# luanaruiz9/gated_gcrnns

Measured on AMD Instinct MI355X. Metric: sequences/sec (node), N=1000 K=5 T=32 F=64, higher is better.
Workload: dtype bf16

## Files before the change

### gated_gcrnns_amd/csrc/gcrnn_fused_seq32.h

```cpp
#pragma once

#if defined(GCRNN_SEQ_STAMPS)
static __device__ unsigned long long gcrnn_seq32_stamps[256 * 96];
static __device__ __forceinline__ void gcrnn_stamp32_put(uint32_t lds_addr) {
  const unsigned long long tv = __builtin_amdgcn_s_memtime();
  asm volatile("ds_write_b64 %0, %1" ::"v"(lds_addr), "v"(tv) : "memory");
}
static __device__ __forceinline__ unsigned long long gcrnn_stamp32_get(uint32_t lds_addr) {
  unsigned long long tv;
  asm volatile("ds_read_b64 %0, %1\n\ts_waitcnt lgkmcnt(0)" : "=v"(tv) : "v"(lds_addr) : "memory");
  return tv;
}
#define GCRNN_STAMP32(slot)                                                                                   \
  do {                                                                                                        \
    if (wave == 0 && stamp_on && lane_now() == 0) gcrnn_stamp32_put((uint32_t)reinterpret_cast<uintptr_t>(smem) + M::FLAG_OFF + 8 * (slot)); \
  } while (0)
#define GCRNN_STAMP32_WAVE(slot0)                                                                             \
  do {                                                                                                        \
    if (stamp_on && lane_now() == 0) gcrnn_stamp32_put((uint32_t)reinterpret_cast<uintptr_t>(smem) + M::FLAG_OFF + 8 * ((slot0) + wave)); \
  } while (0)
#define GCRNN_STAMP32_FLUSH()                                                                                 \
  do {                                                                                                        \
    __syncthreads();                                                                                          \
    if (threadIdx.x < 96 && blockIdx.x < 256) gcrnn_seq32_stamps[blockIdx.x * 96 + threadIdx.x] = gcrnn_stamp32_get((uint32_t)reinterpret_cast<uintptr_t>(smem) + M::FLAG_OFF + 8 * threadIdx.x); \
// ... 197 lines not shown
          const bool ok = nodes[i] < N;
          const int nn = ok ? nodes[i] : 0;
          const char* ra = smem + (8 * qo) * SROW + ((((nn >> 3) + 2 * qo) & 127) << 4) + (nn & 7) * 2;
          uint32_t h16[8];
#pragma unroll
          for (int j = 0; j < 8; ++j) h16[j] = *reinterpret_cast<const uint16_t*>(ra + j * SROW);
          typedef __attribute__((__vector_size__(4 * sizeof(unsigned int)))) unsigned int u32x4s_t;
          u32x4s_t v;
#pragma unroll
          for (int jj = 0; jj < 4; ++jj) v[jj] = ok ? (h16[2 * jj] | (h16[2 * jj + 1] << 16)) : 0u;
          bfr[i][s] = __builtin_bit_cast(bf16x8, v);
        }
        lds_barrier();
      }
      if (a.nsteps > 1) {
        constexpr int XN = RPH * NPCK, XROWS = G, XPPR = XN / 8, XPCS = XROWS / 8;
        static_assert(XROWS * XN * 2 <= 32 * SROW && (XROWS * XPPR) % STHREADS == 0 && (XPCS * XN) % STHREADS == 0 && XPPR >= 16, "x_1 start-up rounds");
        const __amdgpu_buffer_rsrc_t rsrc_x1 = __builtin_amdgcn_make_buffer_rsrc(a.pk_dst0 + a.pkdst_stride + (int64_t)b * (NP * G), 0, NP * G * 2, 0x00020000);
        const uint16_t* src = a.pk_src0 + (int64_t)b * a.pk_stride + a.pksrc_stride;
#pragma unroll
        for (int i = 0; i < XROWS * XPPR / STHREADS; ++i) {
          const int id = i * STHREADS + tl;
          const int row = id / XPPR, cs = id - row * XPPR;
          const int col = (cs - 2 * (row >> 3) + XPPR) % XPPR;
          if (col * 8 < N)
            __builtin_amdgcn_global_load_lds((const __attribute__((address_space(1))) void*)(src + (int64_t)row * N + col * 8),
                                             (__attribute__((address_space(3))) void*)(smem + (i * STHREADS + wave * 64) * 16), 16, 0, GCRNN_SEQ32_NT_DMA);
        }
        asm volatile("s_waitcnt vmcnt(0)" ::: "memory");
        lds_barrier();
        constexpr int XRI = XPCS * XN / STHREADS;
        typedef __attribute__((__vector_size__(4 * sizeof(unsigned int)))) unsigned int u32x4x_t;
        u32x4x_t vv[XRI];
#pragma unroll
        for (int i = 0; i < XRI; ++i) {
          const int id = i * STHREADS + tl;
          const int nl = id / XPCS, pc = id - nl * XPCS;
          const char* ra = smem + (8 * pc) * (XN * 2) + ((((nl >> 3) + 2 * pc) % XPPR) << 4) + (nl & 7) * 2;
          uint32_t h16[8];
#pragma unroll
          for (int j = 0; j < 8; ++j) h16[j] = *reinterpret_cast<const uint16_t*>(ra + j * (XN * 2));
          const bool ok = nl < N;
#pragma unroll
          for (int jj = 0; jj < 4; ++jj) vv[i][jj] = ok ? (h16[2 * jj] | (h16[2 * jj + 1] << 16)) : 0u;
        }
#pragma unroll
        for (int i = 0; i < XRI; ++i) asm volatile("" : "+v"(vv[i]));
#pragma unroll
        for (int i = 0; i < XRI; ++i) {
          const int id = i * STHREADS + tl;
          const int nl = id / XPCS, pc = id - nl * XPCS;
          __builtin_amdgcn_raw_buffer_store_b128(vv[i], rsrc_x1, nl * (G * 2) + pc * 16, 0, 0);
        }
        asm volatile("s_waitcnt vmcnt(0)" ::: "memory");
#pragma unroll
        for (int i = 0; i < XRI; ++i) asm volatile("" ::"v"(vv[i]));
        lds_barrier();
      }
    }
  }

  int tbeg[STILES], tend[STILES];
#pragma unroll
  for (int i = 0; i < STILES; ++i) {
    tbeg[i] = a.tile_off[wave * STILES + i];
    tend[i] = a.tile_off[wave * STILES + i + 1];
  }
  char* wtab = smem + COL_OFF + entries * 32 + GCRNN_HOP_COLUMN_PAD;
  for (int idx = tid; idx < NP; idx += STHREADS) reinterpret_cast<int32_t*>(wtab)[idx] = a.tile_nodes[idx];
  [[maybe_unused]] float* r1tab = reinterpret_cast<float*>(wtab + NP * 4);
  if constexpr (R1) {
    for (int idx = tid; idx < NP; idx += STHREADS) {
      const int nd = a.tile_nodes[idx] >> 16;
      r1tab[idx] = nd < NP ? a.r1a[nd] : 0.f;
      r1tab[NP + idx] = nd < NP ? a.r1b[nd] : 0.f;
    }
  }
  auto slot_words = [&](int ln, int (&w)[STILES]) {
    const uint32_t ad = (uint32_t)(COL_OFF + entries * 32 + GCRNN_HOP_COLUMN_PAD) + (uint32_t)((wave * STILES * 16 + (ln & 15)) * 4);
    asm volatile("ds_read_b32 %0, %8\n\tds_read_b32 %1, %8 offset:64\n\tds_read_b32 %2, %8 offset:128\n\tds_read_b32 %3, %8 offset:192\n\t"
                 "ds_read_b32 %4, %8 offset:256\n\tds_read_b32 %5, %8 offset:320\n\tds_read_b32 %6, %8 offset:384\n\tds_read_b32 %7, %8 offset:448\n\t"
                 "s_waitcnt lgkmcnt(0)"
                 : "=&v"(w[0]), "=&v"(w[1]), "=&v"(w[2]), "=&v"(w[3]), "=&v"(w[4]), "=&v"(w[5]), "=&v"(w[6]), "=&v"(w[7])
                 : "v"(ad));
    const int lb = (((ln >> 4) >> 1) << 4) | (((ln >> 4) & 1) << 3);
#pragma unroll
    for (int i = 0; i < STILES; ++i) w[i] ^= lb;
  };
  [[maybe_unused]] auto r1_scale = [&](f32x4 (&ac)[STILES][2], int kind) __attribute__((always_inline)) {
    if constexpr (R1) {
      const uint32_t ad = (uint32_t)(COL_OFF + entries * 32 + GCRNN_HOP_COLUMN_PAD + NP * 4 + NP * 4) + (uint32_t)((wave * STILES * 16 + (lane_now() & 15)) * 4);
      constexpr int NB = (GATED || ITEMS || K == 4) ? 1 : 4;
#pragma unroll
      for (int h4 = 0; h4 < STILES; h4 += NB) {
        float b4[NB];
        if constexpr (NB == 4)
          asm volatile("ds_read_b32 %0, %4\n\tds_read_b32 %1, %4 offset:64\n\tds_read_b32 %2, %4 offset:128\n\tds_read_b32 %3, %4 offset:192\n\t"
                       "s_waitcnt lgkmcnt(0)"
                       : "=&v"(b4[0]), "=&v"(b4[1]), "=&v"(b4[2]), "=&v"(b4[3])
                       : "v"(ad + (uint32_t)(h4 * 64)));
        else
          asm volatile("ds_read_b32 %0, %1\n\ts_waitcnt lgkmcnt(0)" : "=&v"(b4[0]) : "v"(ad + (uint32_t)(h4 * 64)));
#pragma unroll
        for (int e = 0; e < NB; ++e) {
          const float bv = b4[e];
          const float f = kind == 0 ? bv : (bv == 0.f ? 1.f : (kind == 1 ? __builtin_amdgcn_rcpf(bv) : bv));
          ac[h4 + e][0] *= f; ac[h4 + e][1] *= f;
        }
      }
    }
  };

  {
    const int cbytes = entries * 32;
    const char* csrc = reinterpret_cast<const char*>(a.ell_col4);
    for (int p = wave; p * 1024 < cbytes; p += SWAVES)
      if (p * 1024 + lane * 16 < cbytes)
        __builtin_amdgcn_global_load_lds((const __attribute__((address_space(1))) void*)(csrc + p * 1024 + lane * 16),
                                         (__attribute__((address_space(3))) void*)(smem + COL_OFF + p * 1024), 16, 0, 0);
    const char* wsrc = reinterpret_cast<const char*>(a.wpack) + (size_t)chunk0 * WB;
    for (int p = wave; p < WB / 1024; p += SWAVES)
      __builtin_amdgcn_global_load_lds((const __attribute__((address_space(1))) void*)(wsrc + p * 1024 + lane * 16),
                                       (__attribute__((address_space(3))) void*)(smem + WOFF + p * 1024), 16, 0, 0);
    asm volatile("s_waitcnt vmcnt(0)" ::: "memory");
  }
  if (tid < GCRNN_HOP_COLUMN_PAD / 4) reinterpret_cast<uint32_t*>(smem + COL_OFF + entries * 32)[tid] = 0u;
  float* lbias = reinterpret_cast<float*>(smem + M::BIAS_OFF);
  if constexpr (UPR1) {
    if (tid < F) lbias[tid] = a.head_w[tid];
  } else
  if (tid < NCH * 32) lbias[tid] = a.bias ? a.bias[tid] : 0.f;
  if constexpr (HEADV) {
    float* ht = reinterpret_cast<float*>(smem + COL_OFF + entries * 32 + GCRNN_HOP_COLUMN_PAD + NP * 4 + (R1 ? 2 * NP * 4 : 0));
    if (tid < F) ht[tid] = a.head_w[tid];
    if (tid == F) ht[64] = a.head_b ? a.head_b[0] : 0.f;
  }
  __syncthreads();

  if (a.stagger > 0) {
    const unsigned long long t0 = __builtin_amdgcn_s_memtime();
    const unsigned long long d = (unsigned long long)((blockIdx.x >> 3) & 7) * (unsigned long long)a.stagger;
    while (__builtin_amdgcn_s_memtime() - t0 < d) __builtin_amdgcn_s_sleep(16);
  }
  const uint32_t lds0 = (uint32_t)reinterpret_cast<uintptr_t>(smem);
  if (lds0 != 0) __builtin_trap();
  const uint32_t lds_col = lds0 + COL_OFF;
  [[maybe_unused]] float* htab = reinterpret_cast<float*>(wtab + NP * 4 + (R1 ? 2 * NP * 4 : 0));
  char* xtile = wtab + NP * 4 + (R1 ? 2 * NP * 4 : 0) + (HEADV ? M::HEAD_TAB : 0);

  const int skip_hi = __builtin_amdgcn_readfirstlane((MODE == 3 || (MODE == 1 && a.flags && a.flags[0] != 0)) ? 1 : 0);
  const bool skip_h = skip_hi != 0;
  auto load_first_operand = [&](int b) {
    const __amdgpu_buffer_rsrc_t rsrc_h = __builtin_amdgcn_make_buffer_rsrc(const_cast<uint16_t*>(a.hfirst), 0, skip_h ? 0 : (ITEMS ? a.hmod : B) * (NP * F * 2), 0x00020000);
    const __amdgpu_buffer_rsrc_t rsrc_x = __builtin_amdgcn_make_buffer_rsrc(const_cast<uint16_t*>(a.x0), 0, XS > 0 ? B * (NP * G * 2) : 0, 0x00020000);
    const int bh = ITEMS ? __builtin_amdgcn_readfirstlane(b % a.hmod) : b;
    const int ln0 = lane_now(), qo = ln0 >> 4;
    int sw[STILES];
    slot_words(ln0, sw);
#pragma unroll
    for (int s = 0; s < KS; ++s) {
#pragma unroll
      for (int i = 0; i < STILES; ++i) {
        const int w = sw[i];
        if (s < HS)
          bfr[i][s] = __builtin_bit_cast(bf16x8, __builtin_amdgcn_raw_buffer_load_b128(rsrc_h, (w >> 16) * (F * 2) + 16 * qo + 64 * s, bh * (NP * F * 2), 0));
        else
          bfr[i][s] = __builtin_bit_cast(bf16x8, __builtin_amdgcn_raw_buffer_load_b128(rsrc_x, (w >> 16) * (G * 2) + 16 * qo + 64 * (s - HS), b * (NP * G * 2), 0));
      }
    }
  };
  bool have_operand = self_start;
  for (int b = wg_seq; b < B; b += gseq) {
  if (!have_operand) load_first_operand(b);
  have_operand = false;
#pragma unroll 1
  for (int step = 0; step < a.nsteps; ++step) {
    const bool fin = (MODE == 2) && a.final_raw && step == a.nsteps - 1;
    uint16_t* hout = fin ? a.final_out : (a.out0 ? a.out0 + (int64_t)step * a.ostride : nullptr);
    [[maybe_unused]] const uint16_t* ep_dh = (SONLY && !fin && a.dh0_) ? a.dh0_ + (int64_t)step * a.dhstride : nullptr;
    [[maybe_unused]] const float* ep_ng = (MODE == 4) ? a.ng0 + (int64_t)step * a.ngstride : nullptr;
    [[maybe_unused]] const uint16_t* ep_h = (MODE == 2) ? (fin ? a.final_h : (a.hs0 ? a.hs0 + (int64_t)step * a.hsstride : nullptr)) : nullptr;
    [[maybe_unused]] const uint16_t* ep_dy = (UPR1 && !fin && a.dy0) ? a.dy0 + (int64_t)step * a.dystride + (int64_t)b * a.dybstride : nullptr;
    [[maybe_unused]] const bool ep_up = UPR1 ? ep_dy != nullptr : ep_dh != nullptr;
    [[maybe_unused]] float* gpart = (MODE == 2 && a.gpart0) ? a.gpart0 + (int64_t)step * a.gpartstride : nullptr;
    [[maybe_unused]] float gsc = 1.f;
    if constexpr (MODE == 2) {
      if (a.gsc0) gsc = __builtin_bit_cast(float, __builtin_amdgcn_readfirstlane(__builtin_bit_cast(int, a.gsc0[(int64_t)step * a.gscstride + b])));
    }
    float gin = 1.f, gfo = 1.f, gratio = 1.f;
    if constexpr (MODE == 4) {
      if (a.gi0) {
        gin = __builtin_bit_cast(float, __builtin_amdgcn_readfirstlane(__builtin_bit_cast(int, a.gi0[(int64_t)step * a.gstride + b])));
        gfo = __builtin_bit_cast(float, __builtin_amdgcn_readfirstlane(__builtin_bit_cast(int, a.gf0[(int64_t)step * a.gstride + b])));
      }
    }
    if constexpr (GATED) {
      gin = __builtin_bit_cast(float, __builtin_amdgcn_readfirstlane(__builtin_bit_cast(int, a.gi0[(int64_t)step * a.gstride + b])));
      gfo = __builtin_bit_cast(float, __builtin_amdgcn_readfirstlane(__builtin_bit_cast(int, a.gf0[(int64_t)step * a.gstride + b])));
      gratio = __builtin_bit_cast(float, __builtin_amdgcn_readfirstlane(__builtin_bit_cast(int, gfo / fmaxf(gin, 1e-30f))));
    }
    const uint16_t* aux1 = (USERV && a.a1) ? (a.a1_last_only ? (step == a.nsteps - 1 ? a.a1 : nullptr) : a.a1 + (int64_t)step * a.a1stride) : nullptr;
    const bool pk_any = PKV && a.pk_src0 != nullptr;
    const int ubstride = a.ubstride;
    const int nb = b + (int)gridDim.x;
    const int nbq = ITEMS ? __builtin_amdgcn_readfirstlane(nb / a.hmod) : 0, nbr = ITEMS ? __builtin_amdgcn_readfirstlane(nb - nbq * a.hmod) : 0;
    const int64_t pk_soff = ITEMS ? (int64_t)nbr * a.pk_stride + (int64_t)nbq * a.pksrc_stride : (int64_t)b * a.pk_stride;
    const int pk_db = ITEMS ? nb : b;
    const __amdgpu_buffer_rsrc_t rsrc_o = __builtin_amdgcn_make_buffer_rsrc(hout, 0, hout ? B * (NP * F * 2) : 0, 0x00020000);
    [[maybe_unused]] const bool stamp_on = (step == (a.nsteps > 2 ? a.nsteps - 3 : 0)) && b == wg_seq;
    GCRNN_STAMP32(0);
    const bool more = step + 1 < a.nsteps;
    const __amdgpu_buffer_rsrc_t rsrc_xn = __builtin_amdgcn_make_buffer_rsrc(const_cast<uint16_t*>(XS > 0 ? a.x0 + (int64_t)(step + 1) * a.xstride : nullptr), 0, (more && XS > 0) ? B * (NP * G * 2) : 0, 0x00020000);

    f32x4 acc[STILES][2];
    auto taps = [&](int tap, [[maybe_unused]] bool on_sums = false) {
#ifdef GCRNN_SEQ32_EXPERIMENT_NO_HOP_TAPS
      if (tap != K - 1) return;
#endif
      const int ln = lane_now();
      const uint32_t wofs = (uint32_t)WOFF + (uint32_t)ln * 16u;
      if constexpr (GATED) {
        const bool xpart = gin > 1e-30f;
        const bool hpart = !on_sums || gfo > 1e-30f;
        if (on_sums) {
          const float pre = hpart ? 1.f / gfo : (xpart ? 1.f / gin : 1.f);
#pragma unroll
          for (int i = 0; i < STILES; ++i) { acc[i][0] *= pre; acc[i][1] *= pre; }
        }
#pragma unroll
        for (int h = 0; h < 2; ++h) {
          if (hpart) {
#pragma unroll
            for (int s = 0; s < HS; ++s) {
              const bf16x8 afr = __builtin_bit_cast(bf16x8, *reinterpret_cast<const uint4*>(smem + wofs + (uint32_t)(((tap * 2 + h) * KS + s) * 1024)));
#pragma unroll
              for (int i = 0; i < STILES; ++i) acc[i][h] = __builtin_amdgcn_mfma_f32_16x16x32_bf16(afr, bfr[i][s], acc[i][h], 0, 0, 0);
            }
          }
          if (hpart) {
#pragma unroll
            for (int i = 0; i < STILES; ++i) acc[i][h] *= (xpart ? gratio : gfo);
          }
          if (xpart) {
#pragma unroll
            for (int s = HS; s < KS; ++s) {
              const bf16x8 afr = __builtin_bit_cast(bf16x8, *reinterpret_cast<const uint4*>(smem + wofs + (uint32_t)(((tap * 2 + h) * KS + s) * 1024)));
#pragma unroll
              for (int i = 0; i < STILES; ++i) acc[i][h] = __builtin_amdgcn_mfma_f32_16x16x32_bf16(afr, bfr[i][s], acc[i][h], 0, 0, 0);
            }
            if constexpr (GATED) {
#pragma unroll
              for (int i = 0; i < STILES; ++i) acc[i][h] *= gin;
            }
          }
        }
      } else if constexpr (ITEMS) {
#pragma unroll
        for (int h = 0; h < 2; ++h)
#pragma unroll
          for (int s = 0; s < KS; ++s) {
            if (s < HS && skip_h) continue;
            const bf16x8 afr = __builtin_bit_cast(bf16x8, *reinterpret_cast<const uint4*>(smem + wofs + (uint32_t)(((tap * 2 + h) * KS + s) * 1024)));
#pragma unroll
            for (int i = 0; i < STILES; ++i) acc[i][h] = __builtin_amdgcn_mfma_f32_16x16x32_bf16(afr, bfr[i][s], acc[i][h], 0, 0, 0);
          }
      } else {
      uint4 af[2];
      af[0] = *reinterpret_cast<const uint4*>(smem + wofs + (uint32_t)((tap * 2 * KS) * 1024));
#pragma unroll
      for (int hs = 0; hs < 2 * KS; ++hs) {
        const int h = hs / KS, s = hs - h * KS;
        if (hs + 1 < 2 * KS) af[(hs + 1) & 1] = *reinterpret_cast<const uint4*>(smem + wofs + (uint32_t)((tap * 2 * KS + hs + 1) * 1024));
        const bf16x8 afr = __builtin_bit_cast(bf16x8, af[hs & 1]);
#pragma unroll
        for (int i = 0; i < STILES; ++i) acc[i][h] = __builtin_amdgcn_mfma_f32_16x16x32_bf16(afr, bfr[i][s], acc[i][h], 0, 0, 0);
      }
      }
    };
    auto put = [&](auto tpc) __attribute__((always_inline)) {
      constexpr bool tprime = decltype(tpc)::value;
      int sw[STILES];
      slot_words(lane_now(), sw);
#pragma unroll
      for (int i = 0; i < STILES; ++i) {
        const int wv = sw[i];
        if constexpr (R1) {
          const int slot = (wave * STILES + i) * 16 + (lane_now() & 15);
          float av = r1tab[slot];
          if constexpr (tprime) { const float bv = r1tab[NP + slot]; av *= (bv == 0.f ? 1.f : bv); }
          state_put<true>(reinterpret_cast<float*>(smem), wv, acc[i][0] * av);
          state_put<true>(reinterpret_cast<float*>(smem + PL), wv, acc[i][1] * av);
        } else {
          state_put<true>(reinterpret_cast<float*>(smem), wv, acc[i][0]);
          state_put<true>(reinterpret_cast<float*>(smem + PL), wv, acc[i][1]);
        }
      }
    };
    auto seed = [&]() {
#pragma unroll
      for (int i = 0; i < STILES; ++i) { acc[i][0] = f32x4{0.f, 0.f, 0.f, 0.f}; acc[i][1] = f32x4{0.f, 0.f, 0.f, 0.f}; }
      taps(K - 1);
      put(std::false_type{});
    };
    seed();

#pragma unroll 1
    for (int chunk = chunk0; chunk < (SPLIT ? chunk0 + 1 : NCH); ++chunk) {
      const bool last = SPLIT || chunk == NCH - 1;
      lds_barrier();
      GCRNN_STAMP32(1 + chunk * 24);

      auto pack_target = [&](int v, int& tgt, int& rnd) -> bool {
        if constexpr (ITEMS) {
          rnd = v; tgt = 0;
          return pk_any && v < NRND && nb < B;
        }
        if constexpr (SPLIT) {
          rnd = v; tgt = 0;
          return pk_any && v < NRND;
        }
        if constexpr (MODE == 2) {
          rnd = v; tgt = step + 1;
          return pk_any && v < NRND && tgt < a.nsteps - (a.final_raw ? 1 : 0);
        }
        v += RPH;
        const int wrap = v >= NRND ? 1 : 0;
        rnd = v - wrap * NRND;
        tgt = step + 1 + wrap;
        return pk_any && tgt >= (self_start ? 1 : 2) && tgt < a.nsteps;
      };
      auto pack_issue = [&](int v) {
        int tgt, rnd;
        if (!pack_target(v, tgt, rnd)) return;
        const uint16_t* pk_src = a.pk_src0 + ((ITEMS || SPLIT) ? 0 : (int64_t)tgt * a.pksrc_stride);
        constexpr int PPR = NPCK / 8, PIECES = PKROWS * PPR;
        static_assert(PIECES % STHREADS == 0, "whole pieces per thread");
        const uint16_t* xsrc = pk_src + pk_soff + rnd * NPCK;
        const int tl = wave * 64 + lane_now();
#pragma unroll
        for (int i = 0; i < PIECES / STHREADS; ++i) {
          const int id = i * STHREADS + tl;
          const int row = id / PPR, cs = id - row * PPR;
          const int col = (cs - (row >> 3)) & (PPR - 1);
          if (rnd * NPCK + col * 8 < N)
            __builtin_amdgcn_global_load_lds((const __attribute__((address_space(1))) void*)(xsrc + (int64_t)row * N + col * 8),
                                             (__attribute__((address_space(3))) void*)(xtile + (i * STHREADS + wave * 64) * 16), 16, 0, GCRNN_SEQ32_NT_DMA);
        }
      };
      auto pack_drain = [&](int v) {
        int tgt, rnd;
        if (!pack_target(v, tgt, rnd)) return;
        uint16_t* pk_dst = a.pk_dst0 + ((ITEMS || SPLIT) ? 0 : (int64_t)tgt * a.pkdst_stride);
        constexpr int PCS = PKROWS / 8, RI = PCS * NPCK / STHREADS;
        static_assert(PCS * NPCK % STHREADS == 0, "whole row pieces per thread");
        typedef __attribute__((__vector_size__(4 * sizeof(unsigned int)))) unsigned int u32x4_t;
        const __amdgpu_buffer_rsrc_t rsrc_pk = __builtin_amdgcn_make_buffer_rsrc(pk_dst, 0, B * (NP * PKROWS * 2), 0x00020000);
        const int tl = wave * 64 + lane_now();
        u32x4_t vv[RI];
        static_assert(RI == 1 || RI == 2, "one or two row pieces per thread");
        uint32_t h16[RI][8];
        uint32_t sa[RI];
#pragma unroll
        for (int i = 0; i < RI; ++i) {
          const int id = i * STHREADS + tl;
          const int nl = id / PCS, pc = id - nl * PCS;
          sa[i] = (uint32_t)(xtile - smem) + (uint32_t)((pc * 8) * (NPCK * 2) + ((nl + 8 * pc) & (NPCK - 1)) * 2);
        }
        static_assert(NPCK * 2 == 256, "row pitch of the pack tile in the asm offsets");
        if constexpr (RI == 2) {
          asm volatile("ds_read_u16 %0, %16\n\tds_read_u16 %1, %16 offset:256\n\tds_read_u16 %2, %16 offset:512\n\tds_read_u16 %3, %16 offset:768\n\t"
                       "ds_read_u16 %4, %16 offset:1024\n\tds_read_u16 %5, %16 offset:1280\n\tds_read_u16 %6, %16 offset:1536\n\tds_read_u16 %7, %16 offset:1792\n\t"
                       "ds_read_u16 %8, %17\n\tds_read_u16 %9, %17 offset:256\n\tds_read_u16 %10, %17 offset:512\n\tds_read_u16 %11, %17 offset:768\n\t"
                       "ds_read_u16 %12, %17 offset:1024\n\tds_read_u16 %13, %17 offset:1280\n\tds_read_u16 %14, %17 offset:1536\n\tds_read_u16 %15, %17 offset:1792\n\t"
                       "s_waitcnt lgkmcnt(0)"
                       : "=&v"(h16[0][0]), "=&v"(h16[0][1]), "=&v"(h16[0][2]), "=&v"(h16[0][3]), "=&v"(h16[0][4]), "=&v"(h16[0][5]), "=&v"(h16[0][6]), "=&v"(h16[0][7]),
                         "=&v"(h16[RI - 1][0]), "=&v"(h16[RI - 1][1]), "=&v"(h16[RI - 1][2]), "=&v"(h16[RI - 1][3]), "=&v"(h16[RI - 1][4]), "=&v"(h16[RI - 1][5]), "=&v"(h16[RI - 1][6]), "=&v"(h16[RI - 1][7])
                       : "v"(sa[0]), "v"(sa[RI - 1]));
        } else {
          asm volatile("ds_read_u16 %0, %8\n\tds_read_u16 %1, %8 offset:256\n\tds_read_u16 %2, %8 offset:512\n\tds_read_u16 %3, %8 offset:768\n\t"
                       "ds_read_u16 %4, %8 offset:1024\n\tds_read_u16 %5, %8 offset:1280\n\tds_read_u16 %6, %8 offset:1536\n\tds_read_u16 %7, %8 offset:1792\n\t"
                       "s_waitcnt lgkmcnt(0)"
                       : "=&v"(h16[0][0]), "=&v"(h16[0][1]), "=&v"(h16[0][2]), "=&v"(h16[0][3]), "=&v"(h16[0][4]), "=&v"(h16[0][5]), "=&v"(h16[0][6]), "=&v"(h16[0][7])
                       : "v"(sa[0]));
        }
#pragma unroll
        for (int i = 0; i < RI; ++i) {
          const int id = i * STHREADS + tl;
          const int nl = id / PCS;
          const bool ok = rnd * NPCK + nl < N;
          uint32_t w4[4];
#pragma unroll
          for (int jj = 0; jj < 4; ++jj) w4[jj] = h16[i][2 * jj] | (h16[i][2 * jj + 1] << 16);
          vv[i] = u32x4_t{ok ? w4[0] : 0u, ok ? w4[1] : 0u, ok ? w4[2] : 0u, ok ? w4[3] : 0u};
        }
#pragma unroll
        for (int i = 0; i < RI; ++i) asm volatile("" : "+v"(vv[i]));
#pragma unroll
        for (int i = 0; i < RI; ++i) {
          const int id = i * STHREADS + tl;
          const int nl = id / PCS, pc = id - nl * PCS;
          __builtin_amdgcn_raw_buffer_store_b128(vv[i], rsrc_pk, (rnd * NPCK + nl) * (PKROWS * 2) + pc * 16 + pk_db * (NP * PKROWS * 2), 0, 0);
        }
      };

      auto r0_of = [&](int j) { return (chunk * (K - 1) + (j - 1)) * RPH; };
      auto weights_issue = [&](int wc, int tap) {
        const char* wsrc = reinterpret_cast<const char*>(a.wpack) + (size_t)wc * WB + (size_t)tap * (2 * KS * 1024);
        const int lane = lane_now();
#pragma unroll
        for (int i = 0; i < (2 * KS + SWAVES - 1) / SWAVES; ++i) {
          const int piece = i * SWAVES + wave;
          if (piece < 2 * KS)
            __builtin_amdgcn_global_load_lds((const __attribute__((address_space(1))) void*)(wsrc + piece * 1024 + lane * 16),
                                             (__attribute__((address_space(3))) void*)(smem + WOFF + tap * (2 * KS * 1024) + piece * 1024), 16, 0, 0);
        }
      };
      typedef __attribute__((__vector_size__(4 * sizeof(unsigned int)))) unsigned int u32x4e_t;
      [[maybe_unused]] u32x4e_t eph[MODE == 2 ? STILES : 1], epg[(SONLY && !UPR1) ? STILES : 1];
      [[maybe_unused]] uint32_t epy[UPR1 ? STILES : 1];
      [[maybe_unused]] float epn[MODE == 4 ? STILES : 1][2];
#ifndef GCRNN_SEQ32_EP_FIRST
#define GCRNN_SEQ32_EP_FIRST 1
#endif
#ifndef GCRNN_SEQ32_EP_EARLY
#define GCRNN_SEQ32_EP_EARLY 0
#endif
      constexpr int EPH = (SONLY && K >= 4 && !GCRNN_SEQ32_EP_EARLY) ? K - 2 : 0;
      auto ep_request = [&](auto i0c, auto i1c) __attribute__((always_inline)) {
        if constexpr (MODE == 4) {
          constexpr int I0 = decltype(i0c)::value, I1 = decltype(i1c)::value;
          const int lq = lane_now();
          int swp[STILES];
          slot_words(lq, swp);
          const __amdgpu_buffer_rsrc_t rsrc_eg = __builtin_amdgcn_make_buffer_rsrc(const_cast<uint16_t*>(ep_dh), 0, ep_dh ? B * (NP * F * 2) : 0, 0x00020000);
          const __amdgpu_buffer_rsrc_t rsrc_n = __builtin_amdgcn_make_buffer_rsrc(const_cast<float*>(ep_ng), 0, (int)(a.nghalf * 8), 0x00020000);
#pragma unroll
          for (int i = I0; i < I1; ++i) {
            const int node = swp[i] >> 16;
            epg[i] = __builtin_amdgcn_raw_buffer_load_b128(rsrc_eg, node * (F * 2) + (chunk * 32 + (lq >> 4) * 8) * 2, b * (NP * F * 2), 0);
            const int go = node < N ? (b * N + node) * 4 : 0x7ffffff0;
            epn[i][0] = __builtin_bit_cast(float, __builtin_amdgcn_raw_buffer_load_b32(rsrc_n, go, 0, 0));
            epn[i][1] = __builtin_bit_cast(float, __builtin_amdgcn_raw_buffer_load_b32(rsrc_n, go, (int)(a.nghalf * 4), 0));
          }
        }
        if constexpr (MODE == 2) {
          constexpr int I0 = decltype(i0c)::value, I1 = decltype(i1c)::value;
          const int lq = lane_now();
          int swp[STILES];
          slot_words(lq, swp);
          const __amdgpu_buffer_rsrc_t rsrc_eh = __builtin_amdgcn_make_buffer_rsrc(const_cast<uint16_t*>(ep_h), 0, ep_h ? B * (NP * F * 2) : 0, 0x00020000);
          const __amdgpu_buffer_rsrc_t rsrc_eg = UPR1 ? __builtin_amdgcn_make_buffer_rsrc(const_cast<uint16_t*>(ep_dy), 0, ep_dy ? N * 2 : 0, 0x00020000)
                                                      : __builtin_amdgcn_make_buffer_rsrc(const_cast<uint16_t*>(ep_dh), 0, ep_dh ? B * (NP * F * 2) : 0, 0x00020000);
#pragma unroll
          for (int i = I0; i < I1; ++i) {
            const int eoff = (swp[i] >> 16) * (F * 2) + (chunk * 32 + (lq >> 4) * 8) * 2;
            eph[i] = __builtin_amdgcn_raw_buffer_load_b128(rsrc_eh, eoff, b * (NP * F * 2), 0);
            if constexpr (UPR1) epy[i] = __builtin_amdgcn_raw_buffer_load_b16(rsrc_eg, (swp[i] >> 16) * 2, 0, 0);
            else epg[i] = __builtin_amdgcn_raw_buffer_load_b128(rsrc_eg, eoff, b * (NP * F * 2), 0);
          }
        }
      };
      if constexpr (SONLY && EPH == 0) ep_request(std::integral_constant<int, 0>{}, std::integral_constant<int, STILES>{});
      auto hop = [&](auto jc) __attribute__((always_inline)) {
        constexpr int j = decltype(jc)::value;
        auto dma_issue = [&]() {
          if (NCH > 1 && !SPLIT) {
            weights_issue((chunk + 1) % NCH, K - j);
            if (j == 1 && K > 2) weights_issue(chunk, 0);
          }
          if (r0_of(j) < NRND) pack_issue(r0_of(j));
        };
        const int r0 = r0_of(j);
#pragma unroll
        for (int i = 0; i < STILES; ++i) { acc[i][0] = f32x4{0.f, 0.f, 0.f, 0.f}; acc[i][1] = f32x4{0.f, 0.f, 0.f, 0.f}; }
        const bool stream_first = (!GATED || !GCRNN_SEQ32_GATED_TAPS_FIRST) && (wave < SWAVES / 2 || GCRNN_SEQ32_SAME_ORDER || (R1 && GCRNN_SEQ32_R1_STREAM_FIRST));
        if (stream_first) {
          dma_issue();
          GCRNN_HOP_ASM_WIDE32_STREAM(acc);
          r1_scale(acc, 0);
          GCRNN_STAMP32(1 + chunk * 24 + 4 * (j - 1) + 1);
          if (j == 2 && chunk == 0) GCRNN_STAMP32_WAVE(56);
          taps(K - 1 - j, true);
        } else {
          taps(K - 1 - j);
          r1_scale(acc, 1);
          if (j == 2 && chunk == 0) GCRNN_STAMP32_WAVE(56);
          dma_issue();
#if GCRNN_SEQ32_YOUNG_PRIO
          __builtin_amdgcn_s_setprio(GCRNN_SEQ32_YOUNG_PRIO);
#endif
          GCRNN_HOP_ASM_WIDE32_STREAM(acc);
#if GCRNN_SEQ32_YOUNG_PRIO
          __builtin_amdgcn_s_setprio(0);
#endif
        }
        GCRNN_STAMP32(1 + chunk * 24 + 4 * (j - 1) + 2);
        if (j == 2 && chunk == 0) GCRNN_STAMP32_WAVE(64);
        if (pk_any || (NCH > 1 && !SPLIT)) asm volatile("s_waitcnt vmcnt(0)" ::: "memory");
        lds_barrier();
        GCRNN_STAMP32(1 + chunk * 24 + 4 * (j - 1) + 3);
#if GCRNN_SEQ32_EP_FIRST
        if constexpr (SONLY && EPH > 0 && j <= EPH)
          ep_request(std::integral_constant<int, (j - 1) * STILES / (EPH > 0 ? EPH : 1)>{}, std::integral_constant<int, j * STILES / (EPH > 0 ? EPH : 1)>{});
#endif
        if (j < K - 1) {
          if (R1 && !stream_first) put(std::true_type{});
          else put(std::false_type{});
        }
        if constexpr (R1 && j == K - 1) {
          if (!stream_first) r1_scale(acc, 2);
        }
        if (K == 2 && NCH > 1 && !SPLIT) weights_issue((chunk + 1) % NCH, 0);
        if (r0 < NRND) pack_drain(r0);
#pragma unroll
        for (int e = 1; e < RPH; ++e) {
          if (pk_any && r0 + e < NRND) {
            lds_barrier();
            pack_issue(r0 + e);
            asm volatile("s_waitcnt vmcnt(0)" ::: "memory");
            lds_barrier();
            pack_drain(r0 + e);
          }
        }
#if !GCRNN_SEQ32_EP_FIRST
        if constexpr (SONLY && EPH > 0 && j <= EPH)
          ep_request(std::integral_constant<int, (j - 1) * STILES / (EPH > 0 ? EPH : 1)>{}, std::integral_constant<int, j * STILES / (EPH > 0 ? EPH : 1)>{});
#endif
        if (j < K - 1) lds_barrier();
        GCRNN_STAMP32(1 + chunk * 24 + 4 * (j - 1) + 4);
      };
      seq_static_for(hop, std::make_integer_sequence<int, K - 1>{});

      typedef __attribute__((__vector_size__(4 * sizeof(unsigned int)))) unsigned int u32x4_t;
      const int lane = lane_now(), q = lane >> 4, tl = wave * 64 + lane;
      auto scratch_rsrc = [&]() {
        return __builtin_amdgcn_make_buffer_rsrc(SCRV ? a.scr + (int64_t)blockIdx.x * ((HS - 1) * (SCR_CH / 2)) : nullptr, 0, SCRV ? (HS - 1) * SCR_CH : 0, 0x00020000);
      };
      auto request_next_operand = [&]() {
        if (ITEMS || !(last && more)) return;
        const int qo = lane_now() >> 4;
        int sw[STILES];
        slot_words(lane, sw);
        const __amdgpu_buffer_rsrc_t rsrc_hn = __builtin_amdgcn_make_buffer_rsrc(SCRV ? nullptr : hout, 0, SCRV ? 0 : B * (NP * F * 2), 0x00020000);
        [[maybe_unused]] const __amdgpu_buffer_rsrc_t rsrc_sn = scratch_rsrc();
#pragma unroll
        for (int s = 0; s < KS; ++s) {
          if (s == HS - 1) continue;
#pragma unroll
          for (int i = 0; i < STILES; ++i) {
            const int w = sw[i];
#ifdef GCRNN_SEQ32_EXPERIMENT_SKIP
            if ((GCRNN_SEQ32_EXPERIMENT_SKIP == 1) == (s < HS)) continue;
#endif
            if (SCRV && s < HS)
              bfr[i][s] = __builtin_bit_cast(bf16x8, __builtin_amdgcn_raw_buffer_load_b128(rsrc_sn, (lane_now() & 15) * 64 + 16 * qo, s * SCR_CH + (wave * STILES + i) * 1024, 16));
            else if (s < HS)
              bfr[i][s] = __builtin_bit_cast(bf16x8, __builtin_amdgcn_raw_buffer_load_b128(rsrc_hn, (w >> 16) * (F * 2) + 16 * qo + 64 * s, b * (NP * F * 2), GCRNN_SEQ32_NT_XLOAD));
            else
              bfr[i][s] = __builtin_bit_cast(bf16x8, __builtin_amdgcn_raw_buffer_load_b128(rsrc_xn, (w >> 16) * (G * 2) + 16 * qo + 64 * (s - HS), b * (NP * G * 2), GCRNN_SEQ32_NT_XLOAD));
          }
        }
      };
      if (GCRNN_SEQ32_OPERAND_AT == 0) request_next_operand();
      if (ITEMS) GCRNN_STAMP32(1 + chunk * 24 + 19);
      float bs[2][4];
#pragma unroll
      for (int h = 0; h < 2; ++h)
#pragma unroll
        for (int e = 0; e < 4; ++e) bs[h][e] = (MODE >= 3 ? 1.f : (gin + gfo)) * lbias[chunk * 32 + q * 8 + h * 4 + e];
      u32x4_t pkd[STILES];
      int swe[STILES];
      slot_words(lane, swe);
      if constexpr (MODE == 1) {
        const int gate = chunk / HS, cg = chunk - gate * HS;
        if (a.tapf) {
          typedef __attribute__((__vector_size__(4 * sizeof(unsigned int)))) unsigned int u32x4t;
          const uint4* tfp = a.tapf + ((size_t)(gate * HS + cg) * 3) * 64 + lane;
          bf16x8 ta[3];
#pragma unroll
          for (int pl = 0; pl < 3; ++pl) ta[pl] = __builtin_bit_cast(bf16x8, tfp[pl * 64]);
          const __amdgpu_buffer_rsrc_t rsrc_c = __builtin_amdgcn_make_buffer_rsrc(gate ? a.out1 : a.out0, 0, (gate ? a.out1 : a.out0) ? B * (NP * F * 2) : 0, 0x00020000);
          float* so = a.taps_out + (((int64_t)b * 2 + gate) * HS + cg) * (int64_t)a.ntaps * N;
#pragma unroll
          for (int i = 0; i < STILES; ++i) {
            const int node = swe[i] >> 16;
            u32x4t p{0u, 0u, 0u, 0u};
            if (node < N) {
              const f32x4 a0 = acc[i][0], a1 = acc[i][1];
              p[0] = pack2bf(fast_tanh(a0[0] + bs[0][0]), fast_tanh(a0[1] + bs[0][1]));
              p[1] = pack2bf(fast_tanh(a0[2] + bs[0][2]), fast_tanh(a0[3] + bs[0][3]));
              p[2] = pack2bf(fast_tanh(a1[0] + bs[1][0]), fast_tanh(a1[1] + bs[1][1]));
              p[3] = pack2bf(fast_tanh(a1[2] + bs[1][2]), fast_tanh(a1[3] + bs[1][3]));
            }
            if (gate ? a.out1 : a.out0) __builtin_amdgcn_raw_buffer_store_b128(p, rsrc_c, node * (F * 2) + (cg * 32 + q * 8) * 2, b * (NP * F * 2), 0);
            f32x4 d = {0.f, 0.f, 0.f, 0.f};
#pragma unroll
            for (int pl = 2; pl >= 0; --pl) d = __builtin_amdgcn_mfma_f32_16x16x32_bf16(ta[pl], __builtin_bit_cast(bf16x8, p), d, 0, 0, 0);
            if (node < N) {
#pragma unroll
              for (int e = 0; e < 4; ++e)
                if (q * 4 + e < a.ntaps) so[(int64_t)(q * 4 + e) * N + node] = d[e];
            }
          }
        } else {
        const float* gwp = a.gw + (int64_t)gate * N * F + cg * 32 + q * 8;
        uint16_t* cso = gate ? a.out1 : a.out0;
        const __amdgpu_buffer_rsrc_t rsrc_c = __builtin_amdgcn_make_buffer_rsrc(cso, 0, cso ? B * (NP * F * 2) : 0, 0x00020000);
        float part = 0.f;
#ifndef GCRNN_SEQ32_GATE_W_PIPELINE
#define GCRNN_SEQ32_GATE_W_PIPELINE 1
#endif
        float4 w8s[2][2][2];
        auto w8_load = [&](int set, int i0l) __attribute__((always_inline)) {
#pragma unroll
          for (int t2 = 0; t2 < 2; ++t2) {
            const int nd = (swe[i0l + t2] >> 16) < N ? (swe[i0l + t2] >> 16) : N - 1;
            w8s[set][t2][0] = *reinterpret_cast<const float4*>(gwp + (int64_t)nd * F);
            w8s[set][t2][1] = *reinterpret_cast<const float4*>(gwp + (int64_t)nd * F + 4);
          }
        };
        if (GCRNN_SEQ32_GATE_W_PIPELINE) w8_load(0, 0);
#pragma unroll
        for (int i0 = 0; i0 < STILES; i0 += 2) {
          const int wset = GCRNN_SEQ32_GATE_W_PIPELINE ? (i0 >> 1) & 1 : 0;
          if (GCRNN_SEQ32_GATE_W_PIPELINE) { if (i0 + 2 < STILES) w8_load(wset ^ 1, i0 + 2); }
          else w8_load(0, i0);
          const auto& w8 = w8s[wset];
#pragma unroll
          for (int t2 = 0; t2 < 2; ++t2) {
            const int i = i0 + t2;
            const int node = swe[i] >> 16;
            u32x4_t p{0u, 0u, 0u, 0u};
            if (node < N) {
              const f32x4 a0 = acc[i][0], a1 = acc[i][1];
              const float o0 = fast_tanh(a0[0] + bs[0][0]), o1 = fast_tanh(a0[1] + bs[0][1]), o2 = fast_tanh(a0[2] + bs[0][2]), o3 = fast_tanh(a0[3] + bs[0][3]);
              const float o4 = fast_tanh(a1[0] + bs[1][0]), o5 = fast_tanh(a1[1] + bs[1][1]), o6 = fast_tanh(a1[2] + bs[1][2]), o7 = fast_tanh(a1[3] + bs[1][3]);
              part = __builtin_fmaf(o3, w8[t2][0].w, __builtin_fmaf(o2, w8[t2][0].z, __builtin_fmaf(o1, w8[t2][0].y, __builtin_fmaf(o0, w8[t2][0].x, part))));
              part = __builtin_fmaf(o7, w8[t2][1].w, __builtin_fmaf(o6, w8[t2][1].z, __builtin_fmaf(o5, w8[t2][1].y, __builtin_fmaf(o4, w8[t2][1].x, part))));
              p[0] = pack2bf(o0, o1); p[1] = pack2bf(o2, o3); p[2] = pack2bf(o4, o5); p[3] = pack2bf(o6, o7);
            }
            if (cso) __builtin_amdgcn_raw_buffer_store_b128(p, rsrc_c, node * (F * 2) + (cg * 32 + q * 8) * 2, b * (NP * F * 2), 0);
          }
        }
        GCRNN_STAMP32(1 + chunk * 24 + 18);
#pragma unroll
        for (int off = 32; off > 0; off >>= 1) part += __shfl_down(part, off, 64);
        if (lane == 0) a.go[(int64_t)b * (NCH * SWAVES) + chunk * SWAVES + wave] = part;
        }
      } else if constexpr (MODE == 3) {
        const __amdgpu_buffer_rsrc_t rsrc_c = __builtin_amdgcn_make_buffer_rsrc(a.out0, 0, B * (NP * F * 2), 0x00020000);
#pragma unroll
        for (int i = 0; i < STILES; ++i) {
          const int node = swe[i] >> 16;
          u32x4_t p{0u, 0u, 0u, 0u};
          if (node < N) {
            const f32x4 a0 = acc[i][0], a1 = acc[i][1];
            p[0] = pack2bf(a0[0] + bs[0][0], a0[1] + bs[0][1]); p[1] = pack2bf(a0[2] + bs[0][2], a0[3] + bs[0][3]);
            p[2] = pack2bf(a1[0] + bs[1][0], a1[1] + bs[1][1]); p[3] = pack2bf(a1[2] + bs[1][2], a1[3] + bs[1][3]);
          }
          __builtin_amdgcn_raw_buffer_store_b128(p, rsrc_c, node * (F * 2) + (chunk * 32 + q * 8) * 2, b * (NP * F * 2), 0);
        }
      } else if constexpr (MODE == 4) {
#pragma unroll
        for (int i = 0; i < STILES; ++i) {
          const int node = swe[i] >> 16;
          u32x4_t p{0u, 0u, 0u, 0u};
          if (node < N) {
            const float ni = gin * epn[i][0], nf = gfo * epn[i][1];
            float yv[8], rw[8];
#pragma unroll
            for (int e = 0; e < 4; ++e) {
              yv[2 * e] = bf2f((uint16_t)(epg[i][e] & 0xffffu)); yv[2 * e + 1] = bf2f((uint16_t)(epg[i][e] >> 16));
              rw[e] = acc[i][0][e] + bs[0][e]; rw[4 + e] = acc[i][1][e] + bs[1][e];
            }
            float o[8];
#pragma unroll
            for (int e = 0; e < 8; ++e) o[e] = fast_tanh(ni * yv[e] + nf * rw[e]);
            p[0] = pack2bf(o[0], o[1]); p[1] = pack2bf(o[2], o[3]); p[2] = pack2bf(o[4], o[5]); p[3] = pack2bf(o[6], o[7]);
          }
          pkd[i] = p;
          __builtin_amdgcn_raw_buffer_store_b128(p, rsrc_o, node * (F * 2) + (chunk * 32 + q * 8) * 2, b * (NP * F * 2), 0);
        }
      } else if constexpr (MODE == 2) {
        float part = 0.f;
        [[maybe_unused]] float hw8[8];
        if constexpr (UPR1) {
#pragma unroll
          for (int e = 0; e < 8; ++e) hw8[e] = lbias[chunk * 32 + q * 8 + e];
        }
#pragma unroll
        for (int i = 0; i < STILES; ++i) {
          const int node = swe[i] >> 16;
          float hv[8], gv[8], rw[8];
#pragma unroll
          for (int e = 0; e < 4; ++e) {
            hv[2 * e] = bf2f((uint16_t)(eph[i][e] & 0xffffu)); hv[2 * e + 1] = bf2f((uint16_t)(eph[i][e] >> 16));
            if constexpr (!UPR1) { gv[2 * e] = bf2f((uint16_t)(epg[i][e] & 0xffffu)); gv[2 * e + 1] = bf2f((uint16_t)(epg[i][e] >> 16)); }
            rw[e] = acc[i][0][e]; rw[4 + e] = acc[i][1][e];
          }
          if constexpr (UPR1) {
            const float dyv = bf2f((uint16_t)epy[i]);
#pragma unroll
            for (int e = 0; e < 8; ++e) gv[e] = bf2f(f2bf(hw8[e] * dyv));
          }
          if (gpart) {
#pragma unroll
            for (int e = 0; e < 8; ++e) part = __builtin_fmaf(rw[e], hv[e], part);
          }
          float o[8];
#pragma unroll
          for (int e = 0; e < 8; ++e) {
            o[e] = rw[e] * gsc;
            if (ep_up) o[e] = (o[e] + gv[e]) * (1.f - hv[e] * hv[e]);
          }
          u32x4_t p{0u, 0u, 0u, 0u};
          if (node < N) { p[0] = pack2bf(o[0], o[1]); p[1] = pack2bf(o[2], o[3]); p[2] = pack2bf(o[4], o[5]); p[3] = pack2bf(o[6], o[7]); }
          pkd[i] = p;
          __builtin_amdgcn_raw_buffer_store_b128(p, rsrc_o, node * (F * 2) + (chunk * 32 + q * 8) * 2, b * (NP * F * 2), 0);
        }
        if (gpart) {
#pragma unroll
          for (int off = 32; off > 0; off >>= 1) part += __shfl_down(part, off, 64);
          if (lane == 0) gpart[(int64_t)b * (NCH * SWAVES) + chunk * SWAVES + wave] = part;
        }
      } else {
#pragma unroll
      for (int i = 0; i < STILES; ++i) {
        const int node = swe[i] >> 16;
        u32x4_t p{0u, 0u, 0u, 0u};
        if (node < N) {
          const f32x4 a0 = acc[i][0], a1 = acc[i][1];
          p[0] = pack2bf(fast_tanh(a0[0] + bs[0][0]), fast_tanh(a0[1] + bs[0][1]));
          p[1] = pack2bf(fast_tanh(a0[2] + bs[0][2]), fast_tanh(a0[3] + bs[0][3]));
          p[2] = pack2bf(fast_tanh(a1[0] + bs[1][0]), fast_tanh(a1[1] + bs[1][1]));
          p[3] = pack2bf(fast_tanh(a1[2] + bs[1][2]), fast_tanh(a1[3] + bs[1][3]));
        }
        pkd[i] = p;
        if constexpr (HEADV) {
          const float4* hwp = reinterpret_cast<const float4*>(htab + chunk * 32 + q * 8);
          const float4 hw0 = hwp[0], hw1 = hwp[1];
          float ys = __builtin_bit_cast(float, p[0] << 16) * hw0.x;
          ys = __builtin_fmaf(hw0.y, __builtin_bit_cast(float, p[0] & 0xffff0000u), ys);
          ys = __builtin_fmaf(hw0.z, __builtin_bit_cast(float, p[1] << 16), ys);
          ys = __builtin_fmaf(hw0.w, __builtin_bit_cast(float, p[1] & 0xffff0000u), ys);
          ys = __builtin_fmaf(hw1.x, __builtin_bit_cast(float, p[2] << 16), ys);
          ys = __builtin_fmaf(hw1.y, __builtin_bit_cast(float, p[2] & 0xffff0000u), ys);
          ys = __builtin_fmaf(hw1.z, __builtin_bit_cast(float, p[3] << 16), ys);
          ys = __builtin_fmaf(hw1.w, __builtin_bit_cast(float, p[3] & 0xffff0000u), ys);
          ys += __shfl_xor(ys, 16, 64);
          ys += __shfl_xor(ys, 32, 64);
          if (q == 0) {
            float* yp = htab + 128 + (wave * STILES + i) * 16 + lane;
            if (HS > 1 && chunk > 0) ys = *yp + ys;
            if (HS > 1 && !last) *yp = ys;
            if (last && node < N) {
              const __amdgpu_buffer_rsrc_t rsrc_y = __builtin_amdgcn_make_buffer_rsrc(a.y0 + ((int64_t)b * a.nsteps + step) * N, 0, N * 4, 0x00020000);
              __builtin_amdgcn_raw_buffer_store_b32(__builtin_bit_cast(unsigned int, ys + htab[64]), rsrc_y, node * 4, 0, 0);
            }
          }
        }
        if constexpr (SCRV) {
          if (!last) __builtin_amdgcn_raw_buffer_store_b128(p, scratch_rsrc(), (lane & 15) * 64 + 16 * q, chunk * SCR_CH + (wave * STILES + i) * 1024, 0);
        } else
        if (GCRNN_SEQ32_NT_STATE && last) __builtin_amdgcn_raw_buffer_store_b128(p, rsrc_o, node * (F * 2) + (chunk * 32 + q * 8) * 2, b * (NP * F * 2), GCRNN_SEQ32_NT_STATE);
        else __builtin_amdgcn_raw_buffer_store_b128(p, rsrc_o, node * (F * 2) + (chunk * 32 + q * 8) * 2, b * (NP * F * 2), 0);
        static_assert(!SCRV || GCRNN_SEQ32_OPERAND_AT != 3, "state scratch: the per-tile request form reads the state image");
        if (GCRNN_SEQ32_OPERAND_AT == 3 && last && more) {
          const __amdgpu_buffer_rsrc_t rsrc_hn = __builtin_amdgcn_make_buffer_rsrc(hout, 0, B * (NP * F * 2), 0x00020000);
#pragma unroll
          for (int s = 0; s < KS; ++s) {
            if (s == HS - 1) continue;
            if (s < HS)
              bfr[i][s] = __builtin_bit_cast(bf16x8, __builtin_amdgcn_raw_buffer_load_b128(rsrc_hn, node * (F * 2) + 16 * q + 64 * s, b * (NP * F * 2), 0));
            else
              bfr[i][s] = __builtin_bit_cast(bf16x8, __builtin_amdgcn_raw_buffer_load_b128(rsrc_xn, node * (G * 2) + 16 * q + 64 * (s - HS), b * (NP * G * 2), 0));
          }
        }
      }
      }
      GCRNN_STAMP32(1 + chunk * 24 + 17);
      if (!ITEMS && last) {
#pragma unroll
        for (int i = 0; i < STILES; ++i) bfr[i][HS - 1] = __builtin_bit_cast(bf16x8, pkd[i]);
      }
      if (GCRNN_SEQ32_OPERAND_AT == 1) request_next_operand();
      if constexpr (ITEMS) {
        if (last && b + (int)gridDim.x < B && !GCRNN_SEQ32_NO_ITEM_PREFETCH) {
          load_first_operand(b + (int)gridDim.x);
          have_operand = true;
        }
      }
      if (aux1) {
        char* tst = smem;
        int swt[STILES];
        slot_words(lane, swt);
#pragma unroll
        for (int i = 0; i < STILES; ++i) {
          const int node = swt[i] >> 16;
          char* ra = tst + (4 * q) * RS2 + node * 4;
#pragma unroll
          for (int k = 0; k < 4; ++k) *reinterpret_cast<uint32_t*>(ra + k * RS2) = pkd[i][k];
        }
        lds_barrier();
        GCRNN_STAMP32(1 + chunk * 24 + 18);
        const int segs = N >> 3;
        uint16_t* ub = const_cast<uint16_t*>(aux1) + (int64_t)b * ubstride + (int64_t)(chunk * 32) * N;
        const __amdgpu_buffer_rsrc_t rsrc_u = __builtin_amdgcn_make_buffer_rsrc(ub, 0, 32 * N * 2, 0x00020000);
        for (int idx = tl; idx < 16 * segs; idx += STHREADS) {
          const int fp = idx / segs, sg = idx - fp * segs;
          const u32x4_t w0 = *reinterpret_cast<const u32x4_t*>(tst + fp * RS2 + sg * 32);
          const u32x4_t w1 = *reinterpret_cast<const u32x4_t*>(tst + fp * RS2 + sg * 32 + 16);
          const u32x4_t ev = {__builtin_amdgcn_perm(w0[1], w0[0], 0x05040100u), __builtin_amdgcn_perm(w0[3], w0[2], 0x05040100u),
                              __builtin_amdgcn_perm(w1[1], w1[0], 0x05040100u), __builtin_amdgcn_perm(w1[3], w1[2], 0x05040100u)};
          const u32x4_t od = {__builtin_amdgcn_perm(w0[1], w0[0], 0x07060302u), __builtin_amdgcn_perm(w0[3], w0[2], 0x07060302u),
                              __builtin_amdgcn_perm(w1[1], w1[0], 0x07060302u), __builtin_amdgcn_perm(w1[3], w1[2], 0x07060302u)};
          __builtin_amdgcn_raw_buffer_store_b128(ev, rsrc_u, ((2 * fp) * N + sg * 8) * 2, 0, GCRNN_SEQ32_NT_ROWS);
          __builtin_amdgcn_raw_buffer_store_b128(od, rsrc_u, ((2 * fp + 1) * N + sg * 8) * 2, 0, GCRNN_SEQ32_NT_ROWS);
        }
      }
      if (GCRNN_SEQ32_OPERAND_AT == 2) request_next_operand();
      GCRNN_STAMP32(1 + chunk * 24 + 19);
      if (K == 2 && NCH > 1 && !SPLIT) asm volatile("s_waitcnt vmcnt(0)" ::: "memory");
      else if (GCRNN_SEQ32_END_WAIT) asm volatile("s_waitcnt vmcnt(0)" ::: "memory");
      lds_barrier();
      GCRNN_STAMP32(1 + chunk * 24 + 20);
      if (!SPLIT && chunk + 1 < NCH) seed();
    }
  }
  }
  GCRNN_STAMP32_FLUSH();
}
```

Baseline: 165,000.

## Overlap next-chunk seed taps with row stores and unroll row-store loop

Splits the next chunk's seed into a tap computation and a put. Half the waves run the taps before the row-store phase and the other half after it, so the MFMA tap work overlaps the global row stores. The put stays after the barrier. Separately, the strided row-store loop is replaced with a fixed per-wave layout: two feature-pair rows per wave and two 64-segment sweeps, with all LDS reads batched before the perms and stores. This adds a static_assert tying it to 8 waves and N ≤ 1024, and it relies on the taps not touching LDS regions that the row stores read.

Measured after the change: 166,900 (median of 6 runs). 1.01x the previous value.

```diff
diff --git a/gated_gcrnns_amd/csrc/gcrnn_fused_seq32.h b/gated_gcrnns_amd/csrc/gcrnn_fused_seq32.h
--- a/gated_gcrnns_amd/csrc/gcrnn_fused_seq32.h
+++ b/gated_gcrnns_amd/csrc/gcrnn_fused_seq32.h
@@ -523,6 +523,11 @@
       taps(K - 1);
       put(std::false_type{});
     };
+    auto seed_taps_beside_rows = [&]() {
+#pragma unroll
+      for (int i = 0; i < STILES; ++i) { acc[i][0] = f32x4{0.f, 0.f, 0.f, 0.f}; acc[i][1] = f32x4{0.f, 0.f, 0.f, 0.f}; }
+      taps(K - 1);
+    };
     seed();
 
 #pragma unroll 1
@@ -753,7 +758,7 @@
       seq_static_for(hop, std::make_integer_sequence<int, K - 1>{});
 
       typedef __attribute__((__vector_size__(4 * sizeof(unsigned int)))) unsigned int u32x4_t;
-      const int lane = lane_now(), q = lane >> 4, tl = wave * 64 + lane;
+      const int lane = lane_now(), q = lane >> 4;
       auto scratch_rsrc = [&]() {
         return __builtin_amdgcn_make_buffer_rsrc(SCRV ? a.scr + (int64_t)blockIdx.x * ((HS - 1) * (SCR_CH / 2)) : nullptr, 0, SCRV ? (HS - 1) * SCR_CH : 0, 0x00020000);
       };
@@ -1024,28 +1029,57 @@
         }
         lds_barrier();
         GCRNN_STAMP32(1 + chunk * 24 + 18);
+      }
+      constexpr bool OVL = USERV && MODE == 0 && !GATED && !SPLIT;
+      const bool ovl = OVL && chunk + 1 < NCH;
+      if (ovl && wave < SWAVES / 2) {
+        seed_taps_beside_rows();
+        GCRNN_STAMP32(1 + chunk * 24 + 21);
+      }
+      if (aux1) {
+        const char* tst = smem;
         const int segs = N >> 3;
         uint16_t* ub = const_cast<uint16_t*>(aux1) + (int64_t)b * ubstride + (int64_t)(chunk * 32) * N;
         const __amdgpu_buffer_rsrc_t rsrc_u = __builtin_amdgcn_make_buffer_rsrc(ub, 0, 32 * N * 2, 0x00020000);
-        for (int idx = tl; idx < 16 * segs; idx += STHREADS) {
-          const int fp = idx / segs, sg = idx - fp * segs;
-          const u32x4_t w0 = *reinterpret_cast<const u32x4_t*>(tst + fp * RS2 + sg * 32);
-          const u32x4_t w1 = *reinterpret_cast<const u32x4_t*>(tst + fp * RS2 + sg * 32 + 16);
-          const u32x4_t ev = {__builtin_amdgcn_perm(w0[1], w0[0], 0x05040100u), __builtin_amdgcn_perm(w0[3], w0[2], 0x05040100u),
-                              __builtin_amdgcn_perm(w1[1], w1[0], 0x05040100u), __builtin_amdgcn_perm(w1[3], w1[2], 0x05040100u)};
-          const u32x4_t od = {__builtin_amdgcn_perm(w0[1], w0[0], 0x07060302u), __builtin_amdgcn_perm(w0[3], w0[2], 0x07060302u),
-                              __builtin_amdgcn_perm(w1[1], w1[0], 0x07060302u), __builtin_amdgcn_perm(w1[3], w1[2], 0x07060302u)};
-          __builtin_amdgcn_raw_buffer_store_b128(ev, rsrc_u, ((2 * fp) * N + sg * 8) * 2, 0, GCRNN_SEQ32_NT_ROWS);
-          __builtin_amdgcn_raw_buffer_store_b128(od, rsrc_u, ((2 * fp + 1) * N + sg * 8) * 2, 0, GCRNN_SEQ32_NT_ROWS);
-        }
-      }
+        static_assert(SWAVES * 2 == 16 && 128 * 32 <= RS2, "row stores: two feature-pair rows per wave, two sweeps of 64 segments inside a tile row");
+        const int ln = lane_now();
+        const char* rb = tst + (2 * wave) * RS2 + ln * 32;
+        u32x4_t rw[4][2], rv[4][2];
+#pragma unroll
+        for (int p = 0; p < 4; ++p) {
+          rw[p][0] = *reinterpret_cast<const u32x4_t*>(rb + (p & 1) * RS2 + (p >> 1) * 2048);
+          rw[p][1] = *reinterpret_cast<const u32x4_t*>(rb + (p & 1) * RS2 + (p >> 1) * 2048 + 16);
+        }
+#pragma unroll
+        for (int p = 0; p < 4; ++p) {
+          const u32x4_t w0 = rw[p][0], w1 = rw[p][1];
+          rv[p][0] = u32x4_t{__builtin_amdgcn_perm(w0[1], w0[0], 0x05040100u), __builtin_amdgcn_perm(w0[3], w0[2], 0x05040100u),
+                             __builtin_amdgcn_perm(w1[1], w1[0], 0x05040100u), __builtin_amdgcn_perm(w1[3], w1[2], 0x05040100u)};
+          rv[p][1] = u32x4_t{__builtin_amdgcn_perm(w0[1], w0[0], 0x07060302u), __builtin_amdgcn_perm(w0[3], w0[2], 0x07060302u),
+                             __builtin_amdgcn_perm(w1[1], w1[0], 0x07060302u), __builtin_amdgcn_perm(w1[3], w1[2], 0x07060302u)};
+        }
+#pragma unroll
+        for (int p = 0; p < 4; ++p) { asm volatile("" : "+v"(rv[p][0])); asm volatile("" : "+v"(rv[p][1])); }
+#pragma unroll
+        for (int p = 0; p < 4; ++p) {
+          const int fp = 2 * wave + (p & 1), sg = ln + 64 * (p >> 1);
+          if (sg < segs) {
+            __builtin_amdgcn_raw_buffer_store_b128(rv[p][0], rsrc_u, ((2 * fp) * N + sg * 8) * 2, 0, GCRNN_SEQ32_NT_ROWS);
+            __builtin_amdgcn_raw_buffer_store_b128(rv[p][1], rsrc_u, ((2 * fp + 1) * N + sg * 8) * 2, 0, GCRNN_SEQ32_NT_ROWS);
+          }
+        }
+      }
+      if (ovl && wave >= SWAVES / 2) seed_taps_beside_rows();
       if (GCRNN_SEQ32_OPERAND_AT == 2) request_next_operand();
       GCRNN_STAMP32(1 + chunk * 24 + 19);
       if (K == 2 && NCH > 1 && !SPLIT) asm volatile("s_waitcnt vmcnt(0)" ::: "memory");
       else if (GCRNN_SEQ32_END_WAIT) asm volatile("s_waitcnt vmcnt(0)" ::: "memory");
       lds_barrier();
       GCRNN_STAMP32(1 + chunk * 24 + 20);
-      if (!SPLIT && chunk + 1 < NCH) seed();
+      if (!SPLIT && chunk + 1 < NCH) {
+        if (ovl) put(std::false_type{});
+        else seed();
+      }
     }
   }
   }
```
